# snap-research/F8Net

Measured on AMD Instinct MI355X. Metric: images/sec at bs=128 (ResNet-50 INT8), higher is better.
Workload: dtype int8 x int8 -> int32 (exact integer)

## Files before the change

f8net_amd/csrc/f8_net.cpp:

```cpp
#include "../../include/f8net.h"
#include "f8_internal.h"

#include <algorithm>
#include <cstdarg>
#include <cstdio>
#include <cstdlib>
#include <cstring>
#include <new>
#include <variant>
#include <string>
#include <mutex>
#include <vector>

using namespace f8;

namespace {

thread_local std::string g_err;

int fail(int code, const char* fmt, ...) {
    char buf[512];
    va_list ap;
    va_start(ap, fmt);
    vsnprintf(buf, sizeof buf, fmt, ap);
// ... 1703 lines not shown
    st.cluster = true;
    const Node& f1 = ND[tail ? r0.b2 : r0.b0];
    if (!tail) { st.src_t = f1.a; st.src_f = find_form(T[f1.a], FORM_I32, 0, 0); }
    else if (int rc = conv_input_i8(net, f1, &st.src_t, &st.src_f)) return rc;
    else if ((rc = conv_input_i8(net, ND[r0.sc], &st.res_t, &st.res_f))) return rc;
    for (int h : ch) pack_block(net, ND[h].blk, true, st);
    const Tensor& o = T[ND[nd.fused_add].out];
    int out_t = ND[nd.fused_add].out;
    if (nd.pool >= 0) {
        out_t = ND[nd.pool].out;
        if (T[out_t].forms.empty()) add_form(T[out_t], FORM_I32, 0, 0);
    }
    select_outputs(net, out_t, &st.out, extra);
    const double px = (double)o.H * o.W, opx = nd.pool >= 0 ? 1.0 : px, n = (double)ch.size();
    st.bytes_per_img = (tail ? px * (T[st.src_t].Cs + T[st.res_t].Cs) : px * o.Cs * 4) + out_bytes(st, o, opx);
    st.valu_per_img = px * ((n - (tail ? 1 : 0)) * o.C * 3.0 + n * o.C * 2.0 + (n - 1) * o.C * 3.0) + opx * 3.0 * o.Cs * out_forms8(st) + (nd.pool >= 0 ? px * o.C : 0.0);
    st.name = "basic_cluster_chain_x" + std::to_string(ch.size()) + (tail ? "_ds:" : ":") + tname(net, f1.out) + ".." + tname(net, nd.out) + (nd.pool >= 0 ? "+avgpool" : "");
    return F8_OK;
}

static int emit_chain(f8_net* net, int i, Step& st, std::vector<int>* extra) {
    auto& T = net->tensors; auto& ND = net->nodes;
    const Node& nd = ND[i];
    const std::vector<int>& ch = nd.chain;
    const Block& r0 = ND[ch[0]].blk;
    const bool tail = r0.b0 < 0;
    const bool ds = r0.sc >= 0;
    const Node& a0 = ND[tail ? r0.b4 : r0.b0];
    const Tensor& x = T[ND[ds ? r0.sc : r0.b0].a];
    st.kind = S_CHAIN;
    if (!ds) { st.src_t = a0.a; st.src_f = find_form(x, FORM_I32, 0, 0); }
    else if (int rc = conv_input_i8(net, ND[tail ? r0.sc : r0.b0], &st.src_t, &st.src_f)) return rc;
    else if (tail && (rc = conv_input_i8(net, a0, &st.src2_t, &st.src2_f))) return rc;
    for (int h : ch) pack_block(net, ND[h].blk, true, st);
    int out_t = ND[nd.fused_add].out;
    const Tensor& o = T[out_t];
    if (nd.pool >= 0) {
        out_t = ND[nd.pool].out;
        if (T[out_t].forms.empty()) add_form(T[out_t], FORM_I32, 0, 0);
    }
    select_outputs(net, out_t, &st.out, extra);
    const double px = (double)o.H * o.W, opx = nd.pool >= 0 ? 1.0 : px;
    st.bytes_per_img = (tail ? px * (x.Cs + T[st.src2_t].Cs) : px * x.Cs * (ds ? 1 : 4)) + out_bytes(st, o, opx);
    const double mid = (double)(tail ? a0.cd.cin : a0.cd.cout);
    st.valu_per_img = px * ((double)(ch.size() - (tail ? 1 : 0)) * 2.0 * mid * 3.0 + (double)ch.size() * o.C * 2.0 + (double)(ch.size() - 1) * o.C * 3.0) +
                      opx * 3.0 * o.Cs * out_forms8(st) + (nd.pool >= 0 ? px * o.C : 0.0);
    st.name = "stage_chain_x" + std::to_string(ch.size()) + (tail ? "_tail" : (ds ? "_ds" : "")) + (nd.pool >= 0 ? "+avgpool:" : ":") + tname(net, a0.out) + ".." + tname(net, nd.out);
    return F8_OK;
}

static int emit_fused(f8_net* net, int i, Step& st, std::vector<int>* extra) {
    auto& T = net->tensors; auto& ND = net->nodes;
    const Node& nd = ND[i];
    const Block& r = nd.blk;
    const Node& na = ND[r.b0]; const Node& nb = ND[r.b2]; const Node& ng = ND[r.b4];
    const bool ds = r.sc >= 0;
    const Tensor& x = T[na.a];
    st.kind = S_FUSED;
    st.variant = r.s2 ? V_OPENER : V_BOTTLENECK;
    if (const int rc = conv_input_i8(net, na, &st.src_t, &st.src_f)) return rc;
    pack_block(net, r, false, st);
    if (!ds) { st.res_t = na.a; st.res_f = find_form(x, FORM_I32, 0, 0); }
    join_shifts(T[nd.out].fl - (ds ? T[ng.out].fl : x.fl), &st.acc_shl, &st.res_shl);
    const int out_t = join_output(net, nd, st);
    select_outputs(net, out_t, &st.out, extra);
    const Tensor& o = T[out_t];
    const double px = (double)x.H * x.W, pxo = (double)o.H * o.W;
    st.valu_per_img = 3.0 * (px * na.cd.cout + pxo * nb.cd.cout) + pxo * o.C * 2.0 + 3.0 * pxo * o.Cs * out_forms8(st);
    st.bytes_per_img = px * x.Cs * (ds ? 1 : 1 + 4) + out_bytes(st, o, pxo);
    st.name = std::string(!ds ? "fused_bottleneck_R" : r.s2 ? "fused_opener_s2_R" : "fused_bottleneck_ds_R") + std::to_string(r.R) + ":" +
              block_names(net, r);
    return F8_OK;
}

static int emit_p12(f8_net* net, int i, Step& st, std::vector<int>* extra) {
    auto& T = net->tensors;
    Node& nd = net->nodes[i]; Node& na = net->nodes[nd.blk.b0];
    const Tensor& x = T[na.a];
    st.kind = S_P12;
    st.variant = nd.blk.s2 ? V_OPENER : V_P12;
    if (const int rc = conv_input_i8(net, na, &st.src_t, &st.src_f)) return rc;
    pack_conv_weights(net, na);
    pack_conv_weights(net, nd);
    if (st.variant == V_P12) { pack_frag_weights(net, na); pack_frag_weights(net, nd); }
    st.relu0 = nd.cd.relu;
    select_outputs(net, nd.out, &st.out, extra);
    if (st.out.f32 >= 0) return fail(F8_ERR_UNSUPPORTED, "finalize: the fused 1x1 -> 3x3 launch writes int8 forms only");
    if (st.variant == V_OPENER && (st.out.f8[0] < 0 || st.out.f8[1] >= 0)) return fail(F8_ERR_UNSUPPORTED, "finalize: the stride-2 1x1 -> 3x3 launch writes exactly one int8 form");
    const Tensor& o = T[nd.out];
    const double px = (double)x.H * x.W, pxo = (double)o.H * o.W;
    st.ops_per_img = conv_ops(net, na) + conv_ops(net, nd);
    st.valu_per_img = 3.0 * (px * na.cd.cout + pxo * o.Cs * out_forms8(st));
    st.bytes_per_img = px * x.Cs + out_bytes(st, o, pxo);
    st.bytes_const = weight_bytes(net, na) + weight_bytes(net, nd);
    st.name = std::string(st.variant == V_OPENER ? "fused_opener_s2_p12_R" + std::to_string(nd.blk.R) + ":" : "fused_p12:") + tname(net, na.out) + "+" + tname(net, nd.out);
    return F8_OK;
}

static int emit_irchain(f8_net* net, int i, Step& st, std::vector<int>* extra) {
    auto& T = net->tensors; auto& ND = net->nodes;
    const Node& nd = ND[i];
    const std::vector<int>& ch = nd.chain;
    const Node& fa = ND[ND[ch[0]].blk.b0];
    const Tensor& x = T[fa.a];
    st.kind = S_IRCHAIN;
    if (const int rc = conv_input_i8(net, fa, &st.src_t, &st.src_f)) return rc;
    if (ND[ch[0]].fused_add >= 0) { st.res_t = fa.a; st.res_f = find_form(x, FORM_I32, 0, 0); }
    const double px = (double)x.H * x.W;
    double valu = 0;
    std::string blocks;
    for (size_t k = 0; k < ch.size(); ++k) {
        const Node& c = ND[ch[k]];
        const Block& r = c.blk;
        pack_block(net, r, false, st);
        const int bo = c.fused_add >= 0 ? ND[c.fused_add].out : c.out;
        valu += 3.0 * px * (ND[r.b0].cd.cout + ND[r.b2].cd.cout) + (c.fused_add >= 0 ? 2.0 * px * T[bo].C : 0.0) + (k + 1 < ch.size() ? 3.0 * px * T[bo].Cs : 0.0);
        const std::string& lb = T[bo].label;
        blocks += (k ? "+" : "") + (lb.empty() ? tname(net, bo) : lb.substr(0, lb.find('.')));
    }
    const int out_t = join_output(net, nd, st);
    st.relu0 = nd.cd.relu;
    select_outputs(net, out_t, &st.out, extra);
    const Tensor& o = T[out_t];
    st.bytes_per_img = px * x.Cs + (st.res_t >= 0 ? px * x.Cs * 4 : 0) + out_bytes(st, o, px);
    st.valu_per_img = valu + 3.0 * px * o.Cs * out_forms8(st);
    st.name = "ir_chain_x" + std::to_string(ch.size()) + ":" + blocks;
    return F8_OK;
}

static int emit_ir(f8_net* net, int i, Step& st, std::vector<int>* extra) {
    auto& T = net->tensors; auto& ND = net->nodes;
    const Node& nd = ND[i];
    const Block& r = nd.blk;
    const Node& na = ND[r.b0]; const Node& nb = ND[r.b2];
    const Tensor& x = T[na.a];
    st.kind = S_IR;
    if (const int rc = conv_input_i8(net, na, &st.src_t, &st.src_f)) return rc;
    pack_block(net, r, false, st);
    st.relu0 = nd.cd.relu;
    const int out_t = join_output(net, nd, st);
    if (nd.fused_add >= 0) {
        st.res_t = na.a; st.res_f = find_form(x, FORM_I32, 0, 0);
        join_shifts(T[nd.out].fl - x.fl, &st.acc_shl, &st.res_shl);
    }
    select_outputs(net, out_t, &st.out, extra);
    const Tensor& o = T[out_t];
    const double px = (double)x.H * x.W, pxo = (double)o.H * o.W;
    st.valu_per_img = 3.0 * (px * na.cd.cout + pxo * nb.cd.cout) + (st.res_t >= 0 ? 2.0 * pxo * o.C : 0.0) + 3.0 * pxo * o.Cs * out_forms8(st);
    st.bytes_per_img = px * x.Cs + (st.res_t >= 0 ? px * x.Cs * 4 : 0) + out_bytes(st, o, pxo);
    char kb[200];
    snprintf(kb, sizeof kb, "fused_ir_s%d_%s:", nb.cd.stride, r.G > 1 ? ("G" + std::to_string(r.G)).c_str() : ("R" + std::to_string(r.R)).c_str());
    st.name = kb + block_names(net, r);
    return F8_OK;
}

static int emit_irk(f8_net* net, int i, Step& st, std::vector<int>* extra) {
    auto& T = net->tensors; auto& ND = net->nodes;
    Node& nd = ND[i];
    const Block& r = nd.blk;
    Node& na = ND[r.b0]; Node& nb = ND[r.b2];
    const Tensor& x = T[na.a];
    st.kind = S_IRK;
    if (const int rc = conv_input_i8(net, na, &st.src_t, &st.src_f)) return rc;
    pack_conv_weights(net, na);
    pack_dwk_weights(net, nb);
    pack_conv_weights(net, nd);
    for (const Node* n : {&na, &nb, &nd}) { st.ops_per_img += conv_ops(net, *n); st.bytes_const += weight_bytes(net, *n); }
// ... 472 lines not shown
            if (nd.dual >= 0) {
                const Node& g = ND[nd.dual];
                const Tensor& s2 = T[st.src2_t];
                a.w2 = W8(g.w_off); a.w2_bytes = (uint32_t)((size_t)g.coutP * g.ktot);
                a.bias2 = B32(g.b_off);
                a.sN2 = s2.H * s2.W * s2.Cs; a.sP2 = g.cd.stride * s2.W * s2.Cs; a.sQ2 = g.cd.stride * s2.Cs; a.ktot2 = g.ktot;
            }
            if (reads_frag_weights(st.variant)) a.w = W8(nd.wf_off);
            if (st.variant == V_WSTAT && nd.dual >= 0) a.w2 = W8(ND[nd.dual].wf_off);
            out_formats(a.q);
            switch (st.variant) {
                case V_FC: fc_dense_kernel_name(kb, sizeof kb, a); break;
                case V_POOL: conv1x1_pool_kernel_name(kb, sizeof kb, a, res); break;
                case V_S2WREG: conv3x3s2_wreg_kernel_name(kb, sizeof kb, a); break;
                case V_WSTAT: conv1x1_wstat_kernel_name(kb, sizeof kb, a, st.inst = conv1x1_wstat_inst(a, res, out32, nq, opt.wstat_fast)); break;
                case V_WREG: conv1x1_wreg_kernel_name(kb, sizeof kb, a); break;
                case V_PATCH3X3: conv3x3_patch_kernel_name(kb, sizeof kb, d.cin, a.W, res); break;
                default: conv_kernel_name(kb, sizeof kb, a, nd.tile, st.inst = conv_inst(a, nd.tile, res, nd.dual >= 0, opt.deep_nk));
            }
            st.args = a; break;
        }
        case S_HEAD2: case S_STEMPOOL: {
            const bool h2 = st.kind == S_HEAD2;
            Node& hc = h2 ? ND[nd.blk.b0] : nd;
            const Tensor& sT = T[st.src_t]; const Form& sF = sT.forms[st.src_f];
            StemPoolArgs a{};
            a.w = W8(hc.w_off); a.w_bytes = (uint32_t)((size_t)hc.coutP * hc.ktot);
            a.bias = B32(hc.b_off);
            a.Hp = sF.Hp; a.Wp = sF.Wp; a.org = sF.pad - hc.cd.pad;
            a.raw_kind = -1;
            if (h2) {
                Node& hb = ND[nd.blk.b2];
                const Tensor& oT = T[nd.out];
                a.h2 = head_dws_form(nd) ? 2 : 1;
                a.relu1 = nd.cd.relu ? 1 : 0; a.Cs = oT.Cs;
                a.wd = W8(hb.w_off); a.bd = B32(hb.cc_off);
                a.w1 = W8(nd.w_off); a.b1 = B32(nd.b_off);
                fmt(hb, &a.na); fmt(nd, &a.nb);
                a.Pc = oT.H; a.Qc = oT.W; a.P = oT.H; a.Q = oT.W;
                a.relu0 = 1;
                a.acc_ok = conv_acc_bounded(hc) && conv_acc_bounded(hb) && conv_acc_bounded(nd); a.rq_int = rq_int || !a.acc_ok;
                a.rC = sT.C; a.rH = sT.H; a.rW = sT.W; a.xor8 = sF.sgn ? 0u : 0x80808080u;
            } else {
                const Tensor& cT = T[nd.out]; const Tensor& oT = T[ND[nd.sp_pool].out];
                a.Pc = cT.H; a.Qc = cT.W; a.P = oT.H; a.Q = oT.W;
                a.relu0 = st.relu0;
                a.acc_ok = conv_acc_bounded(nd); a.rq_int = rq_int;
            }
            StemPoolArgs g = a; g.rH = sT.H; g.rW = sT.W;
            st.inst = stem_pool_inst(g, opt.stem_rows, st.raw_input);
            snprintf(kb, sizeof kb, "%s", stem_pool_kernel_name(st.inst));
            out_formats(a.q); st.args = a; break;
        }
        case S_FUSED: {
            const Block& r = nd.blk;
            const bool ds = r.sc >= 0, opener = st.variant == V_OPENER;
            const Node& na = ND[r.b0]; const Node& nb = ND[r.b2]; const Node& ng = ND[r.b4];
            const Tensor& x = T[st.src_t];
            FusedArgs a{};
            a.w0 = W8(na.w_off); a.w0_bytes = (uint32_t)((size_t)na.coutP * na.ktot);
            a.w2 = W8(nb.w_off); a.w2_bytes = (uint32_t)((size_t)nb.coutP * nb.ktot);
            a.w4 = W8(ng.w_off); a.w4_bytes = (uint32_t)((size_t)ng.coutP * ng.ktot);
            a.b0 = B32(na.b_off); a.b2 = B32(nb.b_off); a.b4 = B32(ng.b_off);
            if (ds) {
                a.wsc = W8(nd.w_off); a.wsc_bytes = (uint32_t)((size_t)nd.coutP * nd.ktot); a.bsc = B32(nd.b_off);
                a.COUT = nd.cd.cout; a.stride2 = opener ? 1 : 0;
            }
            a.H = x.H; a.W = x.W; a.C = na.cd.cin; a.MID = na.cd.cout; a.R = r.R;
            a.tiles_per_img = opener ? (x.H / 2) / r.R : (x.H + r.R - 1) / r.R;
            fmt(nb, &a.n1, &a.lo1, &a.hi1, &a.xor1);
            fmt(ng, &a.n2, &a.lo2, &a.hi2, &a.xor2);
            a.relu_a = na.cd.relu; a.relu_b = nb.cd.relu;
            a.acc_shl = st.acc_shl; a.res_shl = st.res_shl; a.relu1 = st.relu1;
            out_formats(a.q);
            if (opener) fused_opener_kernel_name(kb, sizeof kb, a, st.inst = fused_opener_inst(a, opt.opener_stg));
            else fused_bottleneck_kernel_name(kb, sizeof kb, a);
            st.args = a; break;
        }
        case S_P12: {
            Node& na = ND[nd.blk.b0];
            const Tensor& x = T[st.src_t];
            FusedArgs a{};
            const bool opener = st.variant == V_OPENER;
            const size_t w0 = opener ? na.w_off : na.wf_off, w2 = opener ? nd.w_off : nd.wf_off;
            a.w0 = W8(w0); a.w0_bytes = (uint32_t)((size_t)na.coutP * na.ktot);
            a.w2 = W8(w2); a.w2_bytes = (uint32_t)((size_t)nd.coutP * nd.ktot);
            a.b0 = B32(na.b_off); a.b2 = B32(nd.b_off);
            a.H = x.H; a.W = x.W; a.C = na.cd.cin; a.MID = na.cd.cout;
            fmt(nd, &a.n1, &a.lo1, &a.hi1, &a.xor1);
            a.relu_a = na.cd.relu; a.relu_b = nd.cd.relu;
            out_formats(a.q);
            if (opener) {
                a.COUT = 4 * na.cd.cout; a.R = nd.blk.R;
                a.tiles_per_img = (x.H / 2 + a.R - 1) / a.R;
                a.n2 = a.q[0].n; a.lo2 = a.q[0].lo; a.hi2 = a.q[0].hi; a.xor2 = a.q[0].bias_xor;
                a.stride2 = 1; a.p12only = 1; a.acc_ok = conv_acc_bounded(na) && conv_acc_bounded(nd); a.rq_int = rq_int;
                fused_opener_kernel_name(kb, sizeof kb, a, st.inst = fused_opener_inst(a, opt.opener_stg));
            } else fused_p12_kernel_name(kb, sizeof kb, a);
            st.args = a; break;
        }
        case S_CHAIN: {
            const std::vector<int>& ch = nd.chain;
            ChainArgs a{};
            a.nblk = (int)ch.size();
            unsigned shortcut_blocks = 0;
            for (int k = 0; k < a.nblk; ++k) {
                const Node& hh = ND[ch[k]];
                const Block& r = ND[ch[k]].blk;
                const Node& ng = ND[r.b4];
                ChainBlk& B = a.blk[k];
                B.w4 = W8(ng.wf_off); B.b4 = B32(ng.b_off);
                if (r.sc >= 0) { B.wsc = W8(hh.wf_off); B.bsc = B32(hh.b_off); shortcut_blocks |= 1u << k; }
                B.relu1 = ND[hh.fused_add].relu;
                join_shifts(T[hh.out].fl - (r.sc >= 0 ? T[ng.out].fl : T[ND[r.b0].a].fl), &B.acc_shl, &B.res_shl);
                if (r.b0 < 0) {
                    B.nq = B.n1 = B.n2 = 1; B.hiq = B.hi1 = B.hi2 = 255; B.xorq = B.xor1 = B.xor2 = 0x80808080u;
                    B.relu_a = B.relu_b = 1;
                    a.acc_ok = 1; a.stream_ok = stream_bounded(net, ND[hh.fused_add].out) ? 1 : 0; a.rq_int = rq_int;
                    continue;
                }
                Node& na = ND[r.b0]; Node& nb = ND[r.b2];
                B.w0 = W8(na.wf_off); B.w2 = W8(nb.wf_off);
                B.b0 = B32(na.b_off); B.b2 = B32(nb.b_off);
                fmt(na, &B.nq, &B.loq, &B.hiq, &B.xorq);
                fmt(nb, &B.n1, &B.lo1, &B.hi1, &B.xor1);
                fmt(ng, &B.n2, &B.lo2, &B.hi2, &B.xor2);
                B.relu_a = na.cd.relu; B.relu_b = nb.cd.relu;
                if (k == 0) { a.acc_ok = 1; a.rq_int = rq_int; a.stream_ok = (r.sc >= 0 || stream_bounded(net, na.a)) ? 1 : 0; }
                a.acc_ok = a.acc_ok && conv_acc_bounded(na) && conv_acc_bounded(nb);
                a.stream_ok = a.stream_ok && stream_bounded(net, ND[hh.fused_add].out);
            }
            const Node& hf = ND[ch[0]];
            const Block& r0 = ND[ch[0]].blk;
            const bool tail = r0.b0 < 0, ds = r0.sc >= 0;
            const Node& a0 = ND[tail ? r0.b4 : r0.b0];
            const Tensor& oT = T[ND[nd.fused_add].out];
            a.tail = tail ? 1 : 0;
            a.pool = nd.pool >= 0 ? 1 : 0;
            st.C = oT.C; st.MID = tail ? a0.cd.cin : a0.cd.cout; st.H = oT.H; st.W = oT.W; st.cin0 = tail ? hf.cd.cin : a0.cd.cin;
            chain_shape(st.C, st.MID, st.H, st.W, st.cin0, tail, &a.R, &st.wg_per_cu);
            st.cluster = (!ds || tail) && cchain_supported(st.C, st.MID, st.H, st.W, st.cin0, tail);
            a.stack = (net->opt.chain_stack && !st.cluster && chain_stackable(st.C, st.MID, st.H, st.W, st.cin0, tail)) ? 2 : 1;
            st.tiles = (a.stack * st.H + a.R - 1) / a.R;
            out_formats(a.q);
            st.inst = chain_fast(a, shortcut_blocks, nq > 0);
            chain_kernel_name(kb, sizeof kb, st.C, st.MID, st.H, st.W, st.cin0, tail, st.inst);
            st.args = a; break;
        }
        case S_BCHAIN: if (st.cluster) {
            const std::vector<int>& ch = nd.chain;
            BCChainArgs a{};
            a.nblk = (int)ch.size();
            for (int k = 0; k < a.nblk; ++k) {
                const Node& hk = ND[ch[k]];
                const Block& r = ND[ch[k]].blk;
                const Node& c2 = ND[r.b2];
                BChainBlk& B = a.blk[k];
                B.wb = W8(c2.wf_off); B.bb = B32(c2.b_off);
                fmt(c2, &B.n1, &B.lo1, &B.hi1, &B.xor1);
                B.relu1 = ND[hk.fused_add].relu;
                if (r.sc >= 0) {
                    a.tail = 1; a.wsc = W8(hk.wf_off); a.bsc = B32(hk.b_off);
                    B.relu_a = ND[T[c2.a].prod].cd.relu;
                    join_shifts(T[c2.out].fl - T[hk.out].fl, &B.acc_shl, &B.res_shl);
                    continue;
                }
                Node& c1 = ND[r.b0];
// ... 1029 lines not shown
```

f8net_amd/csrc/f8_opener.hip:

```cpp
#include "f8_device.h"
#include <cstdlib>
#include <cstdio>

namespace f8 {

template <int C, int MID, int W, int R, int COUT>
struct OpenerCfg {
    static constexpr int WO = W / 2;
    static constexpr int PR = 2 * R + 1;
    static constexpr int NE = WO + 1, NO = WO;
    static constexpr int PW = NE + NO;
    static constexpr int P1_PX = PR * W, NP1 = (P1_PX + 31) / 32;
    static constexpr int OUT_PX = R * WO, NPO = (OUT_PX + 31) / 32;
    static constexpr int PATCH_BYTES = (PR * PW * MID + 255) / 256 * 256;
    static constexpr int X1_BYTES = NP1 * 32 * 64, W0_BYTES = MID * 64, STAGE1 = X1_BYTES + W0_BYTES;
    static constexpr int MID2_BYTES = NPO * 32 * MID, XS_BYTES = NPO * 32 * C;
    static constexpr int W2B = MID * 64, NS2 = 5;
    static constexpr int REG_B = MID2_BYTES + XS_BYTES + NS2 * W2B;
    static constexpr int REG_A = 2 * STAGE1 > REG_B ? 2 * STAGE1 : REG_B;
    static constexpr int BIAS_INTS = 2 * MID + 2 * COUT;
    static constexpr int LDS_BYTES = PATCH_BYTES + REG_A + BIAS_INTS * 4;
    static constexpr int STAGE3 = 64 * MID + 64 * C;
    static constexpr int STG_BYTES = NPO * 32 * 128;
};

template <int C, int MID, int W, int R, int COUT, bool STG, bool P12 = false, int FQ = 0>
__global__ void __launch_bounds__(512) __attribute__((amdgpu_waves_per_eu(2, 2)))
fused_opener_kernel(const FusedArgs a) {
    using Cfg = OpenerCfg<C, MID, W, R, COUT>;
    constexpr int WO = Cfg::WO, PR = Cfg::PR, NE = Cfg::NE, PW = Cfg::PW;
    constexpr int P1_PX = Cfg::P1_PX, NP1 = Cfg::NP1, OUT_PX = Cfg::OUT_PX, NPO = Cfg::NPO;
    constexpr int CM = MID / 32, CMW = CM / 2, NP1W = (NP1 + 3) / 4;
    constexpr int NK1 = C / 64, NK2 = 9 * (MID / 64), NC3 = COUT / 64, KK3 = MID / 32, KKS = C / 32, CH = MID / 64;
    constexpr int X1_BYTES = Cfg::X1_BYTES, STAGE1 = Cfg::STAGE1, W2B = Cfg::W2B, NS2 = Cfg::NS2, STAGE3 = Cfg::STAGE3;
    static_assert(NPO == 4 && CM % 2 == 0 && NP1 % 4 == 0, "4 pixel-tile groups x 2 channel-tile groups");
    static_assert(MID % 64 == 0 && C % 64 == 0 && COUT % 128 == 0, "K steps of 64 bytes, chunk pairs");
    static_assert(Cfg::LDS_BYTES <= 160 * 1024, "LDS");
    static_assert(2 * STAGE3 <= Cfg::PATCH_BYTES && STAGE3 <= NS2 * W2B, "P3 ring: two stages over the patch, one over the W2 ring");
    static_assert(!STG || (Cfg::PATCH_BYTES - 2 * STAGE3 >= Cfg::STG_BYTES && NS2 * W2B - STAGE3 >= Cfg::STG_BYTES), "staging buffers");
    constexpr int XL1 = X1_BYTES / 16 / 512;
    constexpr int WL0 = (MID * 4 + 511) / 512;
    constexpr int WL4 = 64 * MID / 16 / 512, WLS = 64 * C / 16 / 512, XSL = NPO * 32 * C / 16 / 512;
    static_assert(X1_BYTES % 8192 == 0 && (MID * 4) % 512 == 0 && WL4 >= 1 && WLS >= 1, "every wave issues every DMA instruction (compile-time wait counts)");
    constexpr int L1 = XL1 + WL0, L3 = WL4 + WLS;

    if constexpr (FQ == 1) set_fp_round_nearest_even();
    extern __shared__ __attribute__((aligned(16))) char lds[];
    char* const patch = lds;
    char* const regA = lds + Cfg::PATCH_BYTES;
    char* const mid2 = regA;
    char* const xs = regA + Cfg::MID2_BYTES;
    char* const w2ring = xs + Cfg::XS_BYTES;
    int* const bias_lds = (int*)(regA + Cfg::REG_A);
    auto p3slot = [&](int s) -> char* { return s < 2 ? patch + s * STAGE3 : w2ring; };
    auto stgbuf = [&](int b) -> char* { return b == 0 ? patch + 2 * STAGE3 : w2ring + STAGE3; };

    using S64 = Swz<64>;
    using SM = Swz<MID>;
    using SC = Swz<C>;

    const int tid = threadIdx.x;
    const int lane = tid & 63;
    const int wave = __builtin_amdgcn_readfirstlane(tid >> 6) & 7;
    const int wa = wave >> 1, wb = wave & 1;
    const int l31 = lane & 31, lh = lane >> 5;

    int t;
    {
        const int nwg = gridDim.x, bid = blockIdx.x, xcd = bid & 7, qq = nwg >> 3, rr = nwg & 7;
        t = (xcd < rr ? xcd * (qq + 1) : rr * (qq + 1) + (xcd - rr) * qq) + (bid >> 3);
    }
    const int HO = a.H >> 1;
    const int n = t / a.tiles_per_img, ti = t - n * a.tiles_per_img;
    const int p0 = ti * R;
    const int gp1 = (n * a.H + 2 * p0 - 1) * W;
    const int m_tile = (n * HO + p0) * WO;

    const __amdgpu_buffer_rsrc_t rx = __builtin_amdgcn_make_buffer_rsrc((void*)a.x8, 0, a.x_bytes, 0x00020000);
    const __amdgpu_buffer_rsrc_t rw0 = __builtin_amdgcn_make_buffer_rsrc((void*)a.w0, 0, a.w0_bytes, 0x00020000);
    const __amdgpu_buffer_rsrc_t rw2 = __builtin_amdgcn_make_buffer_rsrc((void*)a.w2, 0, a.w2_bytes, 0x00020000);
    const __amdgpu_buffer_rsrc_t rw4 = __builtin_amdgcn_make_buffer_rsrc((void*)a.w4, 0, a.w4_bytes, 0x00020000);
    const __amdgpu_buffer_rsrc_t rwsc = __builtin_amdgcn_make_buffer_rsrc((void*)a.wsc, 0, a.wsc_bytes, 0x00020000);

#ifdef F8_TRACE
    unsigned long long tt[8]; tt[0] = __builtin_readcyclecounter();
#define F8_OT(i) tt[i] = __builtin_readcyclecounter()
#else
#define F8_OT(i)
#endif

    for (int i = tid; i < (P12 ? 2 * MID : Cfg::BIAS_INTS); i += 512) {
        int v;
        if (i < MID) v = a.b0[i];
        else if (i < 2 * MID) v = a.b2[i - MID];
        else if (i < 2 * MID + COUT) v = a.b4[i - 2 * MID];
        else v = a.bsc[i - 2 * MID - COUT];
        bias_lds[i] = v;
    }
    {
        const unsigned z = a.xor1;
        const v4i zv = {(int)z, (int)z, (int)z, (int)z};
        if (tid < PR * (MID / 16)) *(v4i*)(patch + (tid / (MID / 16)) * PW * MID + (tid % (MID / 16)) * 16) = zv;
        if (p0 == 0)
            for (int o = tid * 16; o < PW * MID; o += 512 * 16) *(v4i*)(patch + o) = zv;
    }

    unsigned xb1[XL1];
#pragma unroll
    for (int i = 0; i < XL1; ++i) {
        const int idx = tid + i * 512;
        const int row = idx >> 2, chunk = (idx & 3) ^ S64::f(row);
        const int pr = row / W;
        const bool ok = row < P1_PX && (2 * p0 - 1 + pr) >= 0;
        xb1[i] = ok ? (unsigned)((gp1 + row) * C + chunk * 16) : kOOB;
    }
    unsigned w0b[WL0], w2b[WL0];
#pragma unroll
    for (int j = 0; j < WL0; ++j) {
        const int idx = tid + j * 512;
        const int row = idx >> 2, chunk = (idx & 3) ^ S64::f(row);
        w0b[j] = (unsigned)(row * C + chunk * 16);
        w2b[j] = (unsigned)(row * (9 * MID) + chunk * 16);
    }
    unsigned w4b[WL4], wsb[WLS], xsb[XSL];
#pragma unroll
    for (int j = 0; j < WL4; ++j) {
        const int idx = tid + j * 512;
        const int row = idx / (MID / 16), c = (idx % (MID / 16)) ^ SM::f(row);
        w4b[j] = (unsigned)(row * MID + c * 16);
    }
#pragma unroll
    for (int j = 0; j < WLS; ++j) {
        const int idx = tid + j * 512;
        const int row = idx / (C / 16), c = (idx % (C / 16)) ^ SC::f(row);
        wsb[j] = (unsigned)(row * C + c * 16);
    }
#pragma unroll
    for (int j = 0; j < XSL; ++j) {
        const int idx = tid + j * 512;
        const int row = idx / (C / 16), c = (idx % (C / 16)) ^ SC::f(row);
        const int orow = row / WO, ocol = row - orow * WO;
        xsb[j] = row < OUT_PX ? (unsigned)(((n * a.H + 2 * (p0 + orow)) * W + 2 * ocol) * C + c * 16) : kOOB;
    }

    auto issue_p1 = [&](int ks, int slot) {
        char* base = regA + slot * STAGE1;
#pragma unroll
        for (int i = 0; i < XL1; ++i) {
            const unsigned off = xb1[i] + (unsigned)(ks * 64);
            __builtin_amdgcn_raw_ptr_buffer_load_lds(rx, (__attribute__((address_space(3))) void*)(base + i * 8192 + wave * 1024), 16, off, 0, 0, 0);
        }
#pragma unroll
        for (int j = 0; j < WL0; ++j) {
            const unsigned woff = w0b[j] + (unsigned)(ks * 64);
            __builtin_amdgcn_raw_ptr_buffer_load_lds(rw0, (__attribute__((address_space(3))) void*)(base + X1_BYTES + j * 8192 + wave * 1024), 16, woff, 0, 0, 0);
        }
    };
    auto issue_w2 = [&](int j2, int slot) {
        char* base = w2ring + slot * W2B;
#pragma unroll
        for (int j = 0; j < WL0; ++j) {
            const unsigned woff = w2b[j] + (unsigned)(j2 * 64);
            __builtin_amdgcn_raw_ptr_buffer_load_lds(rw2, (__attribute__((address_space(3))) void*)(base + j * 8192 + wave * 1024), 16, woff, 0, 0, 0);
        }
    };
    auto issue_xs = [&]() {
#pragma unroll
        for (int j = 0; j < XSL; ++j) {
            const unsigned off = xsb[j];
            __builtin_amdgcn_raw_ptr_buffer_load_lds(rx, (__attribute__((address_space(3))) void*)(xs + j * 8192 + wave * 1024), 16, off, 0, 0, 0);
        }
    };
    auto issue_p3 = [&](int c, int slot) {
        char* base = p3slot(slot);
#pragma unroll
        for (int j = 0; j < WL4; ++j) {
            const unsigned woff = w4b[j] + (unsigned)(c * 64 * MID);
            __builtin_amdgcn_raw_ptr_buffer_load_lds(rw4, (__attribute__((address_space(3))) void*)(base + j * 8192 + wave * 1024), 16, woff, 0, 0, 0);
        }
#pragma unroll
        for (int j = 0; j < WLS; ++j) {
            const unsigned woff = wsb[j] + (unsigned)(c * 64 * C);
            __builtin_amdgcn_raw_ptr_buffer_load_lds(rwsc, (__attribute__((address_space(3))) void*)(base + 64 * MID + j * 8192 + wave * 1024), 16, woff, 0, 0, 0);
        }
    };

    unsigned cof[2];
#pragma unroll
    for (int kk = 0; kk < 2; ++kk) cof[kk] = (unsigned)(((kk * 2 + lh) ^ S64::f(l31)) << 4);

    {
        v16i acc[NP1W][CMW];
#pragma unroll
        for (int i = 0; i < CMW; ++i)
#pragma unroll
            for (int g = 0; g < 4; ++g) {
                v4i bv = {0, 0, 0, 0};
                if constexpr (FQ != 0) bv = *(const v4i*)(a.b0 + (wb * CMW + i) * 32 + 8 * g + 4 * lh);
#pragma unroll
                for (int j = 0; j < NP1W; ++j)
#pragma unroll
                    for (int e = 0; e < 4; ++e) acc[j][i][4 * g + e] = bv[e];
            }
        issue_p1(0, 0);
        static_for<NK1>([&](auto kc) {
            constexpr int KS = decltype(kc)::value;
            wait_vmcnt<0>();
            asm volatile("s_waitcnt lgkmcnt(0)" ::: "memory");
            __builtin_amdgcn_s_barrier();
            if constexpr (KS + 1 < NK1) issue_p1(KS + 1, (KS + 1) & 1);
            const char* base = regA + (KS & 1) * STAGE1;
#pragma unroll
            for (int kk = 0; kk < 2; ++kk) {
                v4i wf[CMW], xf[NP1W];
#pragma unroll
                for (int i = 0; i < CMW; ++i) wf[i] = *(const v4i*)(base + X1_BYTES + ((wb * CMW + i) * 32 + l31) * 64 + cof[kk]);
#pragma unroll
                for (int j = 0; j < NP1W; ++j) xf[j] = *(const v4i*)(base + ((wa + 4 * j) * 32 + l31) * 64 + cof[kk]);
#pragma unroll
                for (int j = 0; j < NP1W; ++j)
#pragma unroll
                    for (int i = 0; i < CMW; ++i) acc[j][i] = __builtin_amdgcn_mfma_i32_32x32x32_i8(wf[i], xf[j], acc[j][i], 0, 0, 0);
            }
        });
        asm volatile("s_waitcnt lgkmcnt(0)" ::: "memory");
        __builtin_amdgcn_s_barrier();
        F8_OT(1);
        if constexpr (!P12) issue_xs();
#pragma unroll
        for (int k = 0; k < NS2 - 1; ++k) issue_w2(k, k);

        const int floor0 = a.relu_a ? 0 : INT32_MIN;
        const float sc1 = FQ == 1 ? requant_u8_scale(a.n1) : 0.0f;
        (void)floor0; (void)sc1;
#pragma unroll
        for (int j = 0; j < NP1W; ++j) {
            const int pix = (wa + 4 * j) * 32 + l31;
            const int pr = pix / W, pc = pix - pr * W + 1;
            const bool ok = pix < P1_PX && (2 * p0 - 1 + pr) >= 0;
            const int ent = pr * PW + ((pc & 1) ? NE + (pc >> 1) : (pc >> 1));
#pragma unroll
            for (int i = 0; i < CMW; ++i) {
                const int ct = wb * CMW + i;
                unsigned d[4];
#pragma unroll
                for (int g = 0; g < 4; ++g) {
                    if constexpr (FQ != 0) {
                        d[g] = requant_u8x4_sel<FQ == 2 ? 2 : 1>(acc[j][i][4 * g], acc[j][i][4 * g + 1], acc[j][i][4 * g + 2], acc[j][i][4 * g + 3], a.n1, sc1) ^ 0x80808080u;
                    } else {
                        const v4i bv = *(const v4i*)(bias_lds + ct * 32 + 8 * g + 4 * lh);
                        int y[4];
#pragma unroll
                        for (int e = 0; e < 4; ++e) y[e] = requant1(max((int)((unsigned)acc[j][i][4 * g + e] + (unsigned)bv[e]), floor0), a.n1, a.lo1, a.hi1);
                        d[g] = pack4(y[0], y[1], y[2], y[3]) ^ a.xor1;
                    }
                }
                auto s0 = __builtin_amdgcn_permlane32_swap(d[0], d[2], false, false);
                auto s1 = __builtin_amdgcn_permlane32_swap(d[1], d[3], false, false);
                if (ok) {
                    v4i o = {(int)s0[0], (int)s0[1], (int)s1[0], (int)s1[1]};
                    *(v4i*)(patch + SM::off(ent, ct * 2 + lh)) = o;
                }
            }
        }
    }
    F8_OT(2);

    const int opix = wa * 32 + l31;
    const bool opix_ok = opix < OUT_PX;
    const int m = m_tile + opix;

    {
        v16i acc[CMW];
        const int oc = opix_ok ? opix : OUT_PX - 1;
// ... 92 lines not shown
            __builtin_amdgcn_s_barrier();
            if constexpr (c + 2 < NC3) issue_p3(c + 2, (c + 2) % 3);
            asm volatile("" ::: "memory");
            if constexpr (c >= 2 && !(c & 1)) { if (stage0) flush_pair(c - 2); }
            if constexpr (c == 0) {
#pragma unroll
                for (int kk = 0; kk < KK3; ++kk) xf[kk] = *(const v4i*)(mid2 + SM::off(opix, kk * 2 + lh));
#pragma unroll
                for (int kk = 0; kk < KKS; ++kk) xsf[kk] = *(const v4i*)(xs + SC::off(opix, kk * 2 + lh));
            }
            const char* base = p3slot(c % 3);
            const int cot = c * 64 + wb * 32;
            v16i acc, acs;
#pragma unroll
            for (int g = 0; g < 4; ++g) {
                const v4i b4v = *(const v4i*)(bias_lds + 2 * MID + cot + 8 * g + 4 * lh);
                const v4i bsv = *(const v4i*)(bias_lds + 2 * MID + COUT + cot + 8 * g + 4 * lh);
#pragma unroll
                for (int e = 0; e < 4; ++e) { acc[4 * g + e] = b4v[e]; acs[4 * g + e] = bsv[e]; }
            }
#pragma unroll
            for (int kk = 0; kk < KK3; ++kk) {
                const v4i wf = *(const v4i*)(base + SM::off(wb * 32 + l31, kk * 2 + lh));
                acc = __builtin_amdgcn_mfma_i32_32x32x32_i8(wf, xf[kk], acc, 0, 0, 0);
            }
#pragma unroll
            for (int kk = 0; kk < KKS; ++kk) {
                const v4i wf = *(const v4i*)(base + 64 * MID + SC::off(wb * 32 + l31, kk * 2 + lh));
                acs = __builtin_amdgcn_mfma_i32_32x32x32_i8(wf, xsf[kk], acs, 0, 0, 0);
            }
            int y[4][4];
#pragma unroll
            for (int g = 0; g < 4; ++g)
#pragma unroll
                for (int e = 0; e < 4; ++e) {
                    const unsigned s = ((unsigned)acs[4 * g + e] << a.acc_shl) + ((unsigned)acc[4 * g + e] << a.res_shl);
                    y[g][e] = max((int)s, floor1);
                }
            if (a.out32 && opix_ok) {
#pragma unroll
                for (int g = 0; g < 4; ++g) {
                    v4i o = {y[g][0], y[g][1], y[g][2], y[g][3]};
                    *(v4i*)(a.out32 + i32t_index(m, cot + 8 * g + 4 * lh, COUT)) = o;
                }
            }
#pragma unroll
            for (int k = 0; k < 2; ++k) {
                if (!a.q[k].ptr) continue;
                unsigned d[4];
#pragma unroll
                for (int g = 0; g < 4; ++g)
                    d[g] = pack4(requant1(y[g][0], a.q[k].n, a.q[k].lo, a.q[k].hi), requant1(y[g][1], a.q[k].n, a.q[k].lo, a.q[k].hi),
                                 requant1(y[g][2], a.q[k].n, a.q[k].lo, a.q[k].hi), requant1(y[g][3], a.q[k].n, a.q[k].lo, a.q[k].hi)) ^ a.q[k].bias_xor;
                auto s0 = __builtin_amdgcn_permlane32_swap(d[0], d[2], false, false);
                auto s1 = __builtin_amdgcn_permlane32_swap(d[1], d[3], false, false);
                const v4i o = {(int)s0[0], (int)s0[1], (int)s1[0], (int)s1[1]};
                if (STG && k == 0) {
                    const int c16 = (c & 1) * 4 + wb * 2 + lh;
                    *(v4i*)(stgbuf((c >> 1) & 1) + opix * 128 + ((c16 ^ (opix & 7)) << 4)) = o;
                } else if (opix_ok) {
                    *(v4i*)(a.q[k].ptr + (size_t)m * COUT + cot + 16 * lh) = o;
                }
            }
        });
        if (stage0) {
            asm volatile("s_waitcnt lgkmcnt(0)" ::: "memory");
            __builtin_amdgcn_s_barrier();
            flush_pair(NC3 - 2);
        }
    }
#ifdef F8_TRACE
    if (a.trace && tid == 0) {
        asm volatile("s_waitcnt vmcnt(0)" ::: "memory");
        tt[5] = __builtin_readcyclecounter();
        unsigned long long* tp = (unsigned long long*)a.trace + (size_t)blockIdx.x * 8;
        for (int i = 0; i < 6; ++i) tp[i] = tt[i];
    }
#endif
}

template <int C, int MID, int W, int R, int COUT, bool STG, bool P12 = false, int FQ = 0>
static hipError_t launch_opener_t(const FusedArgs& a, hipStream_t s) {
    using Cfg = OpenerCfg<C, MID, W, R, COUT>;
    static unsigned long long attr_done = 0; int attr_dev = -1;
    if (!dyn_lds_opted_in(&attr_done, &attr_dev)) {
        hipError_t e = hipFuncSetAttribute((const void*)fused_opener_kernel<C, MID, W, R, COUT, STG, P12, FQ>, hipFuncAttributeMaxDynamicSharedMemorySize, Cfg::LDS_BYTES);
        if (e != hipSuccess) return e;
        if (attr_dev >= 0) attr_done |= 1ull << attr_dev;
    }
    const int grid = a.N * a.tiles_per_img;
#ifdef F8_TRACE
    static unsigned long long* tbuf = nullptr; static int count = 0;
    static const int want = [] { const char* e = getenv("F8_TRACE_OPENER"); return e ? atoi(e) : -1; }();
    FusedArgs b = a;
    const bool tracing = (count++ == want);
    if (tracing) { if (!tbuf) (void)hipMalloc((void**)&tbuf, (size_t)1 << 22); (void)hipMemsetAsync(tbuf, 0, (size_t)grid * 64, s); b.trace = tbuf; }
    hipLaunchKernelGGL((fused_opener_kernel<C, MID, W, R, COUT, STG, P12, FQ>), dim3(grid), dim3(512), Cfg::LDS_BYTES, s, b);
    if (tracing) {
        (void)hipStreamSynchronize(s);
        unsigned long long* h = new unsigned long long[(size_t)grid * 8];
        (void)hipMemcpy(h, tbuf, (size_t)grid * 64, hipMemcpyDeviceToHost);
        double ph[5] = {0, 0, 0, 0, 0}; int n = 0;
        for (int i = 0; i < grid; ++i) { unsigned long long* p = h + (size_t)i * 8; if (!p[5]) continue; ++n; for (int k = 0; k < 5; ++k) ph[k] += (double)(p[k + 1] - p[k]); }
        fprintf(stderr, "[trace opener<%d,%d,%d,%d,%d>] grid %d: avg cycles per WG: P1 loop %.0f | P1 epi %.0f | P2 loop %.0f | P2 epi %.0f | P3 %.0f\n", C, MID, W, R, COUT, grid,
                ph[0] / n, ph[1] / n, ph[2] / n, ph[3] / n, ph[4] / n);
        delete[] h;
    }
    return hipGetLastError();
#else
    hipLaunchKernelGGL((fused_opener_kernel<C, MID, W, R, COUT, STG, P12, FQ>), dim3(grid), dim3(512), Cfg::LDS_BYTES, s, a);
    return hipGetLastError();
#endif
}

int fused_opener_inst(const FusedArgs& a, bool stg) {
    if (!a.p12only) return stg ? 1 : 0;
    const bool fqf = a.relu_a && a.relu_b && a.n1 > 0 && a.n2 > 0 && a.n1 <= 30 && a.n2 <= 30 && a.lo1 == 0 && a.lo2 == 0 && a.hi1 == 255 && a.hi2 == 255 &&
                     a.xor1 == 0x80808080u && a.xor2 == 0x80808080u;
#ifndef F8_OPENER_FQ
#define F8_OPENER_FQ 1
#endif
    return (!fqf || !F8_OPENER_FQ) ? 0 : ((a.rq_int || !a.acc_ok || a.n1 > kRequantU8MaxShift || a.n2 > kRequantU8MaxShift) ? 2 : 1);
}

int fused_opener_kernel_name(char* buf, size_t cap, const FusedArgs& a, int inst) {
    return snprintf(buf, cap, "f8::fused_opener_kernel<%d, %d, %d, %d, %d, %s, %s, %d>", a.C, a.MID, a.W, a.R, a.COUT, !a.p12only && inst ? "true" : "false",
                    a.p12only ? "true" : "false", a.p12only ? inst : 0);
}

hipError_t launch_fused_opener(const FusedArgs& a, int inst, hipStream_t s) {
    if (a.C == 256 && a.MID == 128 && a.COUT == 512 && a.W == 56 && a.R == 4) {
        if (a.p12only) {
            if (!(a.q[0].ptr && !a.q[1].ptr && !a.out32)) return hipErrorInvalidValue;
            const int fq = inst;
            return fq == 1 ? launch_opener_t<256, 128, 56, 4, 512, false, true, 1>(a, s) : fq == 2 ? launch_opener_t<256, 128, 56, 4, 512, false, true, 2>(a, s)
                                                                                               : launch_opener_t<256, 128, 56, 4, 512, false, true, 0>(a, s);
        }
        return inst ? launch_opener_t<256, 128, 56, 4, 512, true>(a, s) : launch_opener_t<256, 128, 56, 4, 512, false>(a, s);
    }
    return hipErrorInvalidValue;
}

bool fused_opener_supported(int C, int MID, int COUT, int H, int W, int* R) {
    if (C == 256 && MID == 128 && COUT == 512 && W == 56 && H % 8 == 0) { *R = 4; return true; }
    return false;
}

}
```

Before: 158,000.

## Hold 1x1 weights in registers for P12 opener and stream pixel tiles per wave

```diff
diff --git a/f8net_amd/csrc/f8_net.cpp b/f8net_amd/csrc/f8_net.cpp
--- a/f8net_amd/csrc/f8_net.cpp
+++ b/f8net_amd/csrc/f8_net.cpp
@@ -1809,7 +1809,8 @@
     if (const int rc = conv_input_i8(net, na, &st.src_t, &st.src_f)) return rc;
     pack_conv_weights(net, na);
     pack_conv_weights(net, nd);
-    if (st.variant == V_P12) { pack_frag_weights(net, na); pack_frag_weights(net, nd); }
+    pack_frag_weights(net, na);
+    if (st.variant == V_P12) pack_frag_weights(net, nd);
     st.relu0 = nd.cd.relu;
     select_outputs(net, nd.out, &st.out, extra);
     if (st.out.f32 >= 0) return fail(F8_ERR_UNSUPPORTED, "finalize: the fused 1x1 -> 3x3 launch writes int8 forms only");
@@ -2448,7 +2449,7 @@
             const Tensor& x = T[st.src_t];
             FusedArgs a{};
             const bool opener = st.variant == V_OPENER;
-            const size_t w0 = opener ? na.w_off : na.wf_off, w2 = opener ? nd.w_off : nd.wf_off;
+            const size_t w0 = na.wf_off, w2 = opener ? nd.w_off : nd.wf_off;
             a.w0 = W8(w0); a.w0_bytes = (uint32_t)((size_t)na.coutP * na.ktot);
             a.w2 = W8(w2); a.w2_bytes = (uint32_t)((size_t)nd.coutP * nd.ktot);
             a.b0 = B32(na.b_off); a.b2 = B32(nd.b_off);
diff --git a/f8net_amd/csrc/f8_opener.hip b/f8net_amd/csrc/f8_opener.hip
--- a/f8net_amd/csrc/f8_opener.hip
+++ b/f8net_amd/csrc/f8_opener.hip
@@ -22,6 +22,9 @@
     static constexpr int LDS_BYTES = PATCH_BYTES + REG_A + BIAS_INTS * 4;
     static constexpr int STAGE3 = 64 * MID + 64 * C;
     static constexpr int STG_BYTES = NPO * 32 * 128;
+    static constexpr int P1S_STAGE = 32 * C, P1S_SLOTS = 11;
+    static constexpr int P12_REG_A = P1S_SLOTS * P1S_STAGE > NS2 * W2B ? P1S_SLOTS * P1S_STAGE : NS2 * W2B;
+    static constexpr int P12_LDS_BYTES = PATCH_BYTES + P12_REG_A + 2 * MID * 4;
 };
 
 template <int C, int MID, int W, int R, int COUT, bool STG, bool P12 = false, int FQ = 0>
@@ -35,7 +38,7 @@
     constexpr int X1_BYTES = Cfg::X1_BYTES, STAGE1 = Cfg::STAGE1, W2B = Cfg::W2B, NS2 = Cfg::NS2, STAGE3 = Cfg::STAGE3;
     static_assert(NPO == 4 && CM % 2 == 0 && NP1 % 4 == 0, "4 pixel-tile groups x 2 channel-tile groups");
     static_assert(MID % 64 == 0 && C % 64 == 0 && COUT % 128 == 0, "K steps of 64 bytes, chunk pairs");
-    static_assert(Cfg::LDS_BYTES <= 160 * 1024, "LDS");
+    static_assert(Cfg::LDS_BYTES <= 160 * 1024 && Cfg::P12_LDS_BYTES <= 160 * 1024, "LDS");
     static_assert(2 * STAGE3 <= Cfg::PATCH_BYTES && STAGE3 <= NS2 * W2B, "P3 ring: two stages over the patch, one over the W2 ring");
     static_assert(!STG || (Cfg::PATCH_BYTES - 2 * STAGE3 >= Cfg::STG_BYTES && NS2 * W2B - STAGE3 >= Cfg::STG_BYTES), "staging buffers");
     constexpr int XL1 = X1_BYTES / 16 / 512;
@@ -50,8 +53,8 @@
     char* const regA = lds + Cfg::PATCH_BYTES;
     char* const mid2 = regA;
     char* const xs = regA + Cfg::MID2_BYTES;
-    char* const w2ring = xs + Cfg::XS_BYTES;
-    int* const bias_lds = (int*)(regA + Cfg::REG_A);
+    char* const w2ring = P12 ? regA : xs + Cfg::XS_BYTES;
+    int* const bias_lds = (int*)(regA + (P12 ? Cfg::P12_REG_A : Cfg::REG_A));
     auto p3slot = [&](int s) -> char* { return s < 2 ? patch + s * STAGE3 : w2ring; };
     auto stgbuf = [&](int b) -> char* { return b == 0 ? patch + 2 * STAGE3 : w2ring + STAGE3; };
 
@@ -89,7 +92,9 @@
 #define F8_OT(i)
 #endif
 
-    for (int i = tid; i < (P12 ? 2 * MID : Cfg::BIAS_INTS); i += 512) {
+    static_assert(2 * MID <= 512, "P12: one bias word per thread");
+    const int bias_p12 = !P12 ? 0 : tid < MID ? a.b0[tid] : tid < 2 * MID ? a.b2[tid - MID] : 0;
+    for (int i = tid; i < (P12 ? 0 : Cfg::BIAS_INTS); i += 512) {
         int v;
         if (i < MID) v = a.b0[i];
         else if (i < 2 * MID) v = a.b2[i - MID];
@@ -189,7 +194,109 @@
 #pragma unroll
     for (int kk = 0; kk < 2; ++kk) cof[kk] = (unsigned)(((kk * 2 + lh) ^ S64::f(l31)) << 4);
 
-    {
+    if constexpr (P12) {
+        constexpr int NQ = C / 32, NSL = Cfg::P1S_SLOTS, SB = Cfg::P1S_STAGE, XLP = SB / 1024;
+        static_assert(NP1 == 16 && CM == 4 && NSL >= 8 && NSL <= 16 && C % 256 == 0, "8 waves x 2 pixel tiles x 2 units of 2 channel tiles");
+        static_assert(Cfg::PATCH_BYTES >= (PR * PW + 1) * MID, "spare patch entry");
+        const bool extra = wave >= 4 && wave < 4 + (NSL - 8);
+        char* const slot0 = regA + wave * SB;
+        char* const slot1 = extra ? regA + (wave + 4) * SB : slot0;
+        v4i wr[CM][NQ];
+#pragma unroll
+        for (int i = 0; i < CM; ++i)
+#pragma unroll
+            for (int q = 0; q < NQ; ++q) wr[i][q] = *(const v4i*)(a.w0 + ((i * NQ + q) * 64 + lane) * 16);
+        asm volatile("" ::: "memory");
+        auto issue_px = [&](int t, char* slot) {
+#pragma unroll
+            for (int i = 0; i < XLP; ++i) {
+                const int idx = i * 64 + lane;
+                const int row = idx / (C / 16), chunk = (idx % (C / 16)) ^ SC::f(row);
+                const int pix = t * 32 + row, pr = pix / W;
+                const bool ok = pix < P1_PX && (2 * p0 - 1 + pr) >= 0;
+                const unsigned off = ok ? (unsigned)((gp1 + pix) * C + chunk * 16) : kOOB;
+                __builtin_amdgcn_raw_ptr_buffer_load_lds(rx, (__attribute__((address_space(3))) void*)(slot + i * 1024), 16, off, 0, 0, 0);
+            }
+        };
+        issue_px(wave, slot0);
+        if (extra) issue_px(wave + 8, slot1);
+        if (tid < 2 * MID) bias_lds[tid] = bias_p12;
+        asm volatile("s_waitcnt lgkmcnt(0)" ::: "memory");
+        __builtin_amdgcn_s_barrier();
+
+        int ent[2];
+#pragma unroll
+        for (int j = 0; j < 2; ++j) {
+            const int pix = (wave + 8 * j) * 32 + l31;
+            const int pr = pix / W, pc = pix - pr * W + 1;
+            const bool ok = pix < P1_PX && (2 * p0 - 1 + pr) >= 0;
+            ent[j] = ok ? pr * PW + ((pc & 1) ? NE + (pc >> 1) : (pc >> 1)) : PR * PW;
+        }
+        const int floor0 = a.relu_a ? 0 : INT32_MIN;
+        const float sc1 = FQ == 1 ? requant_u8_scale(a.n1) : 0.0f;
+        (void)floor0; (void)sc1;
+        v16i acc[CMW];
+        auto epilogue = [&](auto uc) {
+            constexpr int U = decltype(uc)::value;
+#pragma unroll
+            for (int i = 0; i < CMW; ++i) {
+                const int ct = (U & 1) * CMW + i;
+                unsigned d[4];
+#pragma unroll
+                for (int g = 0; g < 4; ++g) {
+                    if constexpr (FQ != 0) {
+                        d[g] = requant_u8x4_sel<FQ == 2 ? 2 : 1>(acc[i][4 * g], acc[i][4 * g + 1], acc[i][4 * g + 2], acc[i][4 * g + 3], a.n1, sc1) ^ 0x80808080u;
+                    } else {
+                        const v4i bv = *(const v4i*)(bias_lds + ct * 32 + 8 * g + 4 * lh);
+                        int y[4];
+#pragma unroll
+                        for (int e = 0; e < 4; ++e) y[e] = requant1(max((int)((unsigned)acc[i][4 * g + e] + (unsigned)bv[e]), floor0), a.n1, a.lo1, a.hi1);
+                        d[g] = pack4(y[0], y[1], y[2], y[3]) ^ a.xor1;
+                    }
+                }
+                auto s0 = __builtin_amdgcn_permlane32_swap(d[0], d[2], false, false);
+                auto s1 = __builtin_amdgcn_permlane32_swap(d[1], d[3], false, false);
+                const v4i o = {(int)s0[0], (int)s0[1], (int)s1[0], (int)s1[1]};
+                *(v4i*)(patch + SM::off(ent[U / 2], ct * 2 + lh)) = o;
+            }
+        };
+        static_for<4>([&](auto uc) {
+            constexpr int U = decltype(uc)::value, T = U / 2, H = U & 1;
+            if constexpr (U == 0) { if (extra) wait_vmcnt<XLP>(); else wait_vmcnt<0>(); }
+            if constexpr (U == 2) wait_vmcnt<0>();
+            const char* const sl = T == 0 ? slot0 : slot1;
+#pragma unroll
+            for (int i = 0; i < CMW; ++i)
+#pragma unroll
+                for (int g = 0; g < 4; ++g) {
+                    v4i bv = {0, 0, 0, 0};
+                    if constexpr (FQ != 0) bv = *(const v4i*)(bias_lds + (H * CMW + i) * 32 + 8 * g + 4 * lh);
+#pragma unroll
+                    for (int e = 0; e < 4; ++e) acc[i][4 * g + e] = bv[e];
+                }
+            v4i xf[NQ];
+            xf[0] = *(const v4i*)(sl + SC::off(l31, lh));
+            xf[1] = *(const v4i*)(sl + SC::off(l31, 2 + lh));
+            static_for<NQ>([&](auto qc) {
+                constexpr int Q = decltype(qc)::value;
+                if constexpr (Q + 2 < NQ) xf[Q + 2] = *(const v4i*)(sl + SC::off(l31, (Q + 2) * 2 + lh));
+#pragma unroll
+                for (int i = 0; i < CMW; ++i) acc[i] = __builtin_amdgcn_mfma_i32_32x32x32_i8(wr[H * CMW + i][Q], xf[Q], acc[i], 0, 0, 0);
+            });
+            if constexpr (U == 1) {
+                asm volatile("s_waitcnt lgkmcnt(0)" ::: "memory");
+                if (!extra) issue_px(wave + 8, slot0);
+            }
+            if constexpr (U == 3) {
+                asm volatile("s_waitcnt lgkmcnt(0)" ::: "memory");
+                __builtin_amdgcn_s_barrier();
+                F8_OT(1);
+#pragma unroll
+                for (int k = 0; k < NS2 - 1; ++k) issue_w2(k, k);
+            }
+            epilogue(uc);
+        });
+    } else {
         v16i acc[NP1W][CMW];
 #pragma unroll
         for (int i = 0; i < CMW; ++i)
@@ -448,9 +555,11 @@
 template <int C, int MID, int W, int R, int COUT, bool STG, bool P12 = false, int FQ = 0>
 static hipError_t launch_opener_t(const FusedArgs& a, hipStream_t s) {
     using Cfg = OpenerCfg<C, MID, W, R, COUT>;
+    constexpr int LDS_BYTES = P12 ? Cfg::P12_LDS_BYTES : Cfg::LDS_BYTES;
+    if (P12 && a.w0_bytes < (uint32_t)(MID * C)) return hipErrorInvalidValue;
     static unsigned long long attr_done = 0; int attr_dev = -1;
     if (!dyn_lds_opted_in(&attr_done, &attr_dev)) {
-        hipError_t e = hipFuncSetAttribute((const void*)fused_opener_kernel<C, MID, W, R, COUT, STG, P12, FQ>, hipFuncAttributeMaxDynamicSharedMemorySize, Cfg::LDS_BYTES);
+        hipError_t e = hipFuncSetAttribute((const void*)fused_opener_kernel<C, MID, W, R, COUT, STG, P12, FQ>, hipFuncAttributeMaxDynamicSharedMemorySize, LDS_BYTES);
         if (e != hipSuccess) return e;
         if (attr_dev >= 0) attr_done |= 1ull << attr_dev;
     }
@@ -461,7 +570,7 @@
     FusedArgs b = a;
     const bool tracing = (count++ == want);
     if (tracing) { if (!tbuf) (void)hipMalloc((void**)&tbuf, (size_t)1 << 22); (void)hipMemsetAsync(tbuf, 0, (size_t)grid * 64, s); b.trace = tbuf; }
-    hipLaunchKernelGGL((fused_opener_kernel<C, MID, W, R, COUT, STG, P12, FQ>), dim3(grid), dim3(512), Cfg::LDS_BYTES, s, b);
+    hipLaunchKernelGGL((fused_opener_kernel<C, MID, W, R, COUT, STG, P12, FQ>), dim3(grid), dim3(512), LDS_BYTES, s, b);
     if (tracing) {
         (void)hipStreamSynchronize(s);
         unsigned long long* h = new unsigned long long[(size_t)grid * 8];
@@ -474,7 +583,7 @@
     }
     return hipGetLastError();
 #else
-    hipLaunchKernelGGL((fused_opener_kernel<C, MID, W, R, COUT, STG, P12, FQ>), dim3(grid), dim3(512), Cfg::LDS_BYTES, s, a);
+    hipLaunchKernelGGL((fused_opener_kernel<C, MID, W, R, COUT, STG, P12, FQ>), dim3(grid), dim3(512), LDS_BYTES, s, a);
     return hipGetLastError();
 #endif
 }
```

New measurement: 157,400. No clear change (-0.3%).
